# Walter0807/MotionBERT

Hardware: AMD Instinct MI355X
Metric: clips/sec [B,243,17,3] DSTformer fwd+bwd (higher is better)
Workload: dtype bf16; 1 GPU; MotionBERT full DSTformer (dim_feat 512, depth 5, 8 heads, mlp_ratio 2) train step: fwd + bwd + AdamW, 64 clips/GPU x T=243 x J=17, random-init weights, pose loss (mpjpe + 0.5 n_mpjpe + 20 velocity, fused kernel), one-launch flat AdamW; global_batch=64, frames=243, parallelism=dp1

## Files before the change

motionbert_amd/csrc/elementwise.hip:

```cpp
#include "mbx_common.h"

static thread_local char g_err[512] = "";
int mbx_set_error(const char* fmt, ...) {
    va_list ap;
    va_start(ap, fmt);
    vsnprintf(g_err, sizeof(g_err), fmt, ap);
    va_end(ap);
    return 1;
}
extern "C" const char* mbx_last_error(void) { return g_err; }

#include <atomic>
static std::atomic<uintptr_t> g_lds_key[512];
static std::atomic<size_t> g_lds_size[512];
int mbx_set_dyn_lds(const void* kernel, size_t bytes, const char* who) {
    if (bytes > 160 * 1024) return mbx_set_error("%s: needs %zu bytes of LDS (> 160 KiB)", who, bytes);
    int dev = 0;
    if (hipGetDevice(&dev) != hipSuccess) dev = 0;
    const uintptr_t key = (reinterpret_cast<uintptr_t>(kernel) << 6) ^ (uintptr_t)(dev + 1);
    int slot = (int)((key * 0x9E3779B97F4A7C15ull) >> 55);
    for (int probe = 0; probe < 512; ++probe, slot = (slot + 1) & 511) {
        uintptr_t k = g_lds_key[slot].load(std::memory_order_acquire);
        if (k == 0 && g_lds_key[slot].compare_exchange_strong(k, key, std::memory_order_acq_rel)) k = key;
        if (k != key) continue;
// ... 280 lines not shown
        const int rpp = 256 / c4n;
        const int blocks = clamp_grid((M + 4 * rpp - 1) / (4 * rpp), 256 * 8);
        int chunk = (M + blocks - 1) / blocks;
        chunk = ((chunk + 4 * rpp - 1) / (4 * rpp)) * (4 * rpp);
        const int grid = (M + chunk - 1) / chunk;
        hipLaunchKernelGGL(embed_fwd_rows_kernel, dim3(grid), dim3(256), 0, (hipStream_t)stream, x, w, b, pos, temp, h, M, T, J, Din, C, chunk);
    } else {
        const int grid = clamp_grid(((size_t)M * (C / 4) + 255) / 256, 256 * 16);
        hipLaunchKernelGGL(embed_fwd_kernel, dim3(grid), dim3(256), 0, (hipStream_t)stream, x, w, b, pos, temp, h, M, T, J, Din, C);
    }
    MBX_LAUNCH_CHECK("embed_fwd");
    return 0;
}

#define EMB_MAXDIN 4
__device__ __forceinline__ float4 embed_dh4(const float* __restrict__ dh, const bf16_t* __restrict__ dh_a, const bf16_t* __restrict__ dh_b, size_t o) {
    if (dh_a == nullptr) return *reinterpret_cast<const float4*>(dh + o);
    float u[4], v[4];
    load4<bf16_t>(dh_a + o, u);
    load4<bf16_t>(dh_b + o, v);
    return make_float4(u[0] + v[0], u[1] + v[1], u[2] + v[2], u[3] + v[3]);
}
__global__ __launch_bounds__(256) void embed_bwd_kernel(const float* __restrict__ dh, const float* __restrict__ x,
                                                        float* __restrict__ dtemp, float* __restrict__ part, int B, int T,
                                                        int J, int Din, int C, const bf16_t* __restrict__ dh_a = nullptr,
                                                        const bf16_t* __restrict__ dh_b = nullptr) {
    __shared__ float4 red[256][1 + EMB_MAXDIN];
    const int t = blockIdx.x;
    const int stride = J * C + C * Din + C;
    float* prow = part + (size_t)t * stride;
    const int nq = C / 4, ns = max(256 / nq, 1);
    for (int q0 = 0; q0 < nq; q0 += 256) {
        const int q = q0 + (int)threadIdx.x % min(nq, 256), sl = (int)threadIdx.x / min(nq, 256);
        const bool act = q < nq && sl < ns;
        const int c = q * 4;
        float4 at = make_float4(0.f, 0.f, 0.f, 0.f), aw[EMB_MAXDIN];
#pragma unroll
        for (int k = 0; k < EMB_MAXDIN; ++k) aw[k] = make_float4(0.f, 0.f, 0.f, 0.f);
        for (int j = 0; j < J; ++j) {
            float4 ap = make_float4(0.f, 0.f, 0.f, 0.f);
            if (act) {
                for (int b0 = sl; b0 < B; b0 += 8 * ns) {
                    float4 g[8];
#pragma unroll
                    for (int u = 0; u < 8; ++u) {
                        const int b = min(b0 + u * ns, B - 1);
                        g[u] = embed_dh4(dh, dh_a, dh_b, (((size_t)b * T + t) * J + j) * C + c);
                    }
#pragma unroll
                    for (int u = 0; u < 8; ++u) {
                        const int b = b0 + u * ns;
                        const float on = b < B ? 1.f : 0.f;
                        const size_t m = ((size_t)min(b, B - 1) * T + t) * J + j;
                        ap.x = fmaf(on, g[u].x, ap.x); ap.y = fmaf(on, g[u].y, ap.y); ap.z = fmaf(on, g[u].z, ap.z); ap.w = fmaf(on, g[u].w, ap.w);
#pragma unroll
                        for (int k = 0; k < EMB_MAXDIN; ++k)
                            if (k < Din) {
                                const float xv = on * x[m * Din + k];
                                aw[k].x = fmaf(g[u].x, xv, aw[k].x); aw[k].y = fmaf(g[u].y, xv, aw[k].y);
                                aw[k].z = fmaf(g[u].z, xv, aw[k].z); aw[k].w = fmaf(g[u].w, xv, aw[k].w);
                            }
                    }
                }
            }
            red[threadIdx.x][0] = ap;
            __syncthreads();
            if (act && sl == 0) {
                for (int s2 = 1; s2 < ns; ++s2) {
                    const float4 o = red[threadIdx.x + s2 * nq][0];
                    ap.x += o.x; ap.y += o.y; ap.z += o.z; ap.w += o.w;
                }
                *reinterpret_cast<float4*>(prow + (size_t)j * C + c) = ap;
                at.x += ap.x; at.y += ap.y; at.z += ap.z; at.w += ap.w;
            }
            __syncthreads();
        }
#pragma unroll
        for (int k = 0; k < EMB_MAXDIN; ++k) red[threadIdx.x][1 + k] = aw[k];
        __syncthreads();
        if (act && sl == 0) {
            *reinterpret_cast<float4*>(dtemp + (size_t)t * C + c) = at;
            *reinterpret_cast<float4*>(prow + (size_t)J * C + (size_t)C * Din + c) = at;
#pragma unroll
            for (int k = 0; k < EMB_MAXDIN; ++k)
                if (k < Din) {
                    float4 w4 = aw[k];
                    for (int s2 = 1; s2 < ns; ++s2) {
                        const float4 o = red[threadIdx.x + s2 * nq][1 + k];
                        w4.x += o.x; w4.y += o.y; w4.z += o.z; w4.w += o.w;
                    }
// ... 20 lines not shown
        for (int k = 0; k < EMB_MAXDIN; ++k) {
            const float s = wave_sum(a[k]);
            if (lane == 0 && k < Din) dx[(size_t)m * Din + k] = s;
        }
    }
}
extern "C" size_t mbx_embed_bwd_ws(int T, int J, int Din, int C) { return (size_t)T * ((size_t)J * C + (size_t)C * Din + C) * sizeof(float); }
static int launch_embed_bwd(const float* dh, const bf16_t* dh_a, const bf16_t* dh_b, const float* x, const float* w, float* dw, float* db,
                            float* dpos, float* dtemp, float* dx, int B, int T, int J, int Din, int C, void* ws, void* stream) {
    MBX_CHECK_ARG((dh || (dh_a && dh_b)) && x && w && dw && db && dpos && dtemp && ws, "embed_bwd: null pointer");
    MBX_CHECK_ARG(Din <= EMB_MAXDIN, "embed_bwd: dim_in %d > %d unsupported", Din, EMB_MAXDIN);
    MBX_CHECK_ARG(B > 0 && T > 0 && J > 0 && C > 0 && C % 4 == 0, "embed_bwd: bad shape (C %% 4 != 0?)");
    hipStream_t s = (hipStream_t)stream;
    float* part = (float*)ws;
    const int stride = J * C + C * Din + C;
    hipLaunchKernelGGL(embed_bwd_kernel, dim3(T), dim3(256), 0, s, dh, x, dtemp, part, B, T, J, Din, C, dh_a, dh_b);
    MBX_LAUNCH_CHECK("embed_bwd");
    if (mbx_launch_colsum(part, T, stride, 0, J * C, dpos, s)) return 1;
    if (mbx_launch_colsum(part, T, stride, J * C, C * Din, dw, s)) return 1;
    if (mbx_launch_colsum(part, T, stride, J * C + C * Din, C, db, s)) return 1;
    if (dx) {
        const int M = B * T * J;
        hipLaunchKernelGGL(embed_bwd_dx_kernel, dim3(clamp_grid((M + 3) / 4, 2048)), dim3(256), 0, s, dh, w, dx, M, Din, C, dh_a, dh_b);
        MBX_LAUNCH_CHECK("embed_bwd_dx");
    }
    return 0;
}
extern "C" int mbx_embed_bwd(const float* dh, const float* x, const float* w, float* dw, float* db, float* dpos,
                             float* dtemp, float* dx, int B, int T, int J, int Din, int C, void* ws, void* stream) {
    MBX_CHECK_ARG(dh, "embed_bwd: null pointer");
    return launch_embed_bwd(dh, nullptr, nullptr, x, w, dw, db, dpos, dtemp, dx, B, T, J, Din, C, ws, stream);
// ... 728 lines not shown
extern "C" int mbx_average_bwd(const float* dh, float* d_st, float* d_ts, void* d_st_t, void* d_ts_t, size_t n,
                               int dtype, void* stream) {
    MBX_CHECK_ARG(dh && d_st && d_ts && d_st_t && d_ts_t && n % 4 == 0, "average_bwd: bad arguments");
    const int grid = clamp_grid((n / 4 + 255) / 256, 4096);
    if (dtype == MBX_BF16)
        hipLaunchKernelGGL(average_bwd_kernel<bf16_t>, dim3(grid), dim3(256), 0, (hipStream_t)stream, dh, d_st, d_ts, (bf16_t*)d_st_t, (bf16_t*)d_ts_t, n / 4);
    else if (dtype == MBX_F32)
        hipLaunchKernelGGL(average_bwd_kernel<float>, dim3(grid), dim3(256), 0, (hipStream_t)stream, dh, d_st, d_ts, (float*)d_st_t, (float*)d_ts_t, n / 4);
    else
        return mbx_set_error("average_bwd: unknown dtype %d", dtype);
    MBX_LAUNCH_CHECK("average_bwd");
    return 0;
}

#define HEAD_MAXD 8
template <int VPL>
__global__ __launch_bounds__(256) void head_fwd_kernel(const float* __restrict__ rep, const float* __restrict__ w,
                                                       const float* __restrict__ b, float* __restrict__ out, int M, int R,
                                                       int Dout) {
    const int lane = threadIdx.x & 63;
    for (int row = blockIdx.x * 4 + (threadIdx.x >> 6); row < M; row += gridDim.x * 4) {
        float v[VPL][4];
        ROW_LOOP(k) {
            const int c = ROW_C(k);
            if (c < R) load4<float>(rep + (size_t)row * R + c, v[k]);
        }
        float mine = 0.f;
        for (int i = 0; i < Dout; ++i) {
            float a = 0.f;
            ROW_LOOP(k) {
                const int c = ROW_C(k);
                if (c < R) {
                    float ww[4];
                    load4<float>(w + (size_t)i * R + c, ww);
#pragma unroll
                    for (int e = 0; e < 4; ++e) a = fmaf(v[k][e], ww[e], a);
                }
            }
            a = wave_sum(a) + b[i];
            if (lane == i) mine = a;
        }
        if (lane < Dout) out[(size_t)row * Dout + lane] = mine;
    }
}
extern "C" int mbx_head_fwd(const float* rep, const float* w, const float* b, float* out, int M, int R, int Dout,
                            void* stream) {
    MBX_CHECK_ARG(rep && w && b && out, "head_fwd: null pointer");
    MBX_CHECK_ARG(M > 0 && R % 4 == 0 && Dout >= 1 && Dout <= HEAD_MAXD, "head_fwd: need R %% 4 == 0 and 1 <= dim_out <= %d", HEAD_MAXD);
    const int grid = clamp_grid((M + 3) / 4, 256 * 8);
    hipStream_t s = (hipStream_t)stream;
    DISPATCH_VPL(vpl_for(R), hipLaunchKernelGGL((head_fwd_kernel<VPL>), dim3(grid), dim3(256), 0, s, rep, w, b, out, M, R, Dout));
    MBX_LAUNCH_CHECK("head_fwd");
    return 0;
}

#define HEAD_BWD_BLOCKS 1024
template <typename T, int VPL>
// ... 3 lines not shown
    extern __shared__ __attribute__((aligned(16))) float lds[];
    const int lane = threadIdx.x & 63, wave = threadIdx.x >> 6;
    const int n = Dout * R + 8;
    float* mine = lds + (size_t)wave * n;
    constexpr int DG = 4;
    for (int i0 = 0; i0 < Dout; i0 += DG) {
        float gw[DG][VPL][4], gbv[DG];
#pragma unroll
        for (int j = 0; j < DG; ++j) {
            gbv[j] = 0.f;
            ROW_LOOP(k) {
#pragma unroll
                for (int e = 0; e < 4; ++e) gw[j][k][e] = 0.f;
            }
        }
        for (int row = blockIdx.x * 4 + wave; row < M; row += gridDim.x * 4) {
            float dvg[DG];
#pragma unroll
            for (int j = 0; j < DG; ++j) dvg[j] = i0 + j < Dout ? dout[(size_t)row * Dout + i0 + j] : 0.f;
#pragma unroll
            for (int j = 0; j < DG; ++j) gbv[j] += dvg[j];
            float dv[HEAD_MAXD];
            if (i0 == 0) {
#pragma unroll
                for (int q = 0; q < HEAD_MAXD; ++q) dv[q] = q < DG ? dvg[q < DG ? q : 0] : (q < Dout ? dout[(size_t)row * Dout + q] : 0.f);
            }
            ROW_LOOP(k) {
                const int c = ROW_C(k);
                if (c < R) {
                    float r[4];
                    load4<float>(rep + (size_t)row * R + c, r);
#pragma unroll
                    for (int j = 0; j < DG; ++j)
#pragma unroll
                        for (int e = 0; e < 4; ++e) gw[j][k][e] = fmaf(dvg[j], r[e], gw[j][k][e]);
                    if (i0 == 0) {
                        float o[4] = {0.f, 0.f, 0.f, 0.f};
#pragma unroll
                        for (int q = 0; q < HEAD_MAXD; ++q) {
                            if (q < Dout) {
                                float ww[4];
                                load4<float>(w + (size_t)q * R + c, ww);
#pragma unroll
                                for (int e = 0; e < 4; ++e) o[e] = fmaf(dv[q], ww[e], o[e]);
                            }
                        }
#pragma unroll
                        for (int e = 0; e < 4; ++e) o[e] *= (1.0f - r[e] * r[e]);
                        store4<T>(dpre + (size_t)row * R + c, o);
                    }
                }
            }
        }
#pragma unroll
        for (int j = 0; j < DG; ++j) {
            if (i0 + j < Dout) {
                ROW_LOOP(k) {
                    const int c = ROW_C(k);
                    if (c < R) store4<float>(mine + (size_t)(i0 + j) * R + c, gw[j][k]);
                }
                if (lane == 0) mine[Dout * R + i0 + j] = gbv[j];
            }
        }
    }
// ... 54 lines not shown
```

motionbert_amd/csrc/gemm_rows_n.hip:

```cpp
#include "mbx_common.h"
#include "lds_stream.h"
#include "mbx_diag.h"

#ifdef MBX_RN_TRACE
__device__ long long* g_rn_trace;
static constexpr int RN_TRACE_SLOTS = 12;
#define RN_TS(slot_) MBX_STAMP(tsr[slot_])
#else
#define RN_TS(slot_) do { } while (0)
#endif
static constexpr int RN_BM = 128;
static constexpr int RN_STAGE = 32 * 1024;
static constexpr int RN_RING = 4 * RN_STAGE;
template <int NT> struct RnGeo {
    static constexpr int N = 32 * NT, KPS = 32 / NT, TRIP = 16 / KPS, NQ = NT / 4;
    static constexpr int LA = NT == 16 ? 4 : 3, TS0 = NT == 16 ? 25 : 1;
};
__host__ __device__ constexpr int rn_cnt(int kps, int trip, int la, int ts0, bool last, int u) {
    int t_lo = 0, t_hi = 0;
    for (int j = 0; j < kps; ++j) { t_lo += ts0 + 4 * j < 27; t_hi += ts0 + 4 * j > 23; }
    const bool t2 = !last || u - 2 + la < trip, t1 = !last || u - 1 + la < trip, t0 = !last || u + la < trip;
    if (u == 0) return 8 + 2 + 6 + (t0 ? t_lo : 0);
    if (u == 1) return 2 + (8 + (t1 ? kps : 0)) + 6 + (t0 ? t_lo : 0);
    return (2 + (t2 ? t_hi : 0)) + (8 + (t1 ? kps : 0)) + (6 + (t0 ? t_lo : 0));
// ... 358 lines not shown
#pragma unroll
    for (int j = 0; j < NQ; ++j) {
#pragma unroll
        for (int r4 = 0; r4 < 8; ++r4) {
            const int rl = 4 * r4 + xr_e;
            const uint4 v = *reinterpret_cast<const uint4*>(rw + j * 32768 + r4 * 4096 + lane_e * 16);
            *reinterpret_cast<uint4*>(xhat_o + (size_t)min(mw + rl, M - 1) * RN_N + j * 128 + ((xp_e ^ (rl & 15)) << 3)) = v;
        }
    }
    if (g_e == 0 && mw + i_e < M) {
        mean_o[mw + i_e] = mu;
        rstd_o[mw + i_e] = rs;
    }
}

extern "C" size_t mbx_rows_n_pack_bytes(int N, int K) { return (size_t)N * K * sizeof(bf16_t); }

extern "C" int mbx_rows_n_pack_many(const int64_t* desc, int n_desc, int N, int max_k, void* stream) {
    MBX_CHECK_ARG(desc && n_desc > 0, "rows_n_pack_many: bad arguments");
    MBX_CHECK_ARG((N == 512 || N == 256) && max_k >= 256 && max_k % 256 == 0, "rows_n_pack_many: N=%d (256 or 512), max_k=%d (%% 256)", N, max_k);
    hipLaunchKernelGGL(rows_n_pack_many_kernel, dim3(((max_k / 16) * (N / 32) + 3) / 4, n_desc), dim3(256), 0, (hipStream_t)stream, desc, N / 32);
    MBX_LAUNCH_CHECK("rows_n_pack_many");
    return 0;
}

#define RN_CHECK_SHAPE(who_)                                                                                         \
    MBX_CHECK_ARG(M > 0 && ((N == 512 && K >= 512) || (N == 256 && K >= 256)) && K % 256 == 0,                      \
                  who_ ": bad shape M=%d N=%d (512 with K >= 512, or 256 with K >= 256) K=%d (%% 256)", M, N, K)

extern "C" int mbx_rows_lnbwd_t(const void* dy, const void* packed, const void* xhat, const float* rstd, const void* dres_t, void* dx_t,
// ... 9 lines not shown
#ifdef MBX_RN_TRACE
    mbx_diag_arm(HIP_SYMBOL(g_rn_trace), (size_t)grid * RN_TRACE_SLOTS * sizeof(long long), (hipStream_t)stream);
#endif
    if (N == 512)
        hipLaunchKernelGGL(rows_n_lnbwd_kernel<16>, dim3(grid), dim3(256), RN_RING + 4 * 8192, (hipStream_t)stream, (const bf16_t*)dy,
                           (const char*)packed, (const bf16_t*)xhat, rstd, (const bf16_t*)dres_t, (bf16_t*)dx_t, M, K);
    else
        hipLaunchKernelGGL(rows_n_lnbwd_kernel<8>, dim3(grid), dim3(256), RN_RING + 4 * 8192, (hipStream_t)stream, (const bf16_t*)dy,
                           (const char*)packed, (const bf16_t*)xhat, rstd, (const bf16_t*)dres_t, (bf16_t*)dx_t, M, K);
    MBX_LAUNCH_CHECK("rows_lnbwd_t");
    return 0;
}

extern "C" int mbx_rows_resid_ln(const void* a, const void* packed, const float* bias, const float* resid, float* y, void* xhat,
                                 float* mean, float* rstd, float eps, int M, int N, int K, void* stream) {
    MBX_CHECK_ARG(a && packed && bias && resid && y && xhat && mean && rstd, "rows_resid_ln: null pointer");
    RN_CHECK_SHAPE("rows_resid_ln");
    MBX_CHECK_ARG((size_t)M * N * 4 < ((size_t)1 << 32), "rows_resid_ln: M=%d rows of %d bytes exceed the 32-bit row offsets of the kernel", M, N * 4);
    MBX_CHECK_ARG((size_t)M * K * 2 < ((size_t)1 << 32), "rows_resid_ln: a of M=%d x K=%d exceeds the 32-bit lane offsets of the kernel", M, K);
    MBX_CHECK_ARG((const void*)y != (const void*)resid && xhat != a, "rows_resid_ln: y aliases resid (or xhat aliases a): rows past M re-read row M - 1 after it was stored");
    const void* kern = N == 512 ? reinterpret_cast<const void*>(rows_n_resid_ln_kernel<16>) : reinterpret_cast<const void*>(rows_n_resid_ln_kernel<8>);
    if (mbx_set_dyn_lds(kern, RN_RING + 4 * 8192, "rows_resid_ln")) return 1;
    if (N == 512)
        hipLaunchKernelGGL(rows_n_resid_ln_kernel<16>, dim3((M + RN_BM - 1) / RN_BM), dim3(256), RN_RING + 4 * 8192, (hipStream_t)stream, (const bf16_t*)a,
                           (const char*)packed, bias, resid, y, (bf16_t*)xhat, mean, rstd, eps, M, K);
    else
        hipLaunchKernelGGL(rows_n_resid_ln_kernel<8>, dim3((M + RN_BM - 1) / RN_BM), dim3(256), RN_RING + 4 * 8192, (hipStream_t)stream, (const bf16_t*)a,
                           (const char*)packed, bias, resid, y, (bf16_t*)xhat, mean, rstd, eps, M, K);
    MBX_LAUNCH_CHECK("rows_resid_ln");
    return 0;
}
```

motionbert_amd/engine.py:

```python
from __future__ import annotations

from collections import namedtuple
from dataclasses import dataclass
from typing import Any, ClassVar, Dict, List, Optional

import os

import torch

EPI_STORE = 0
EPI_GELU = 1
EPI_RESID = 2
EPI_TANH = 3
EPI_DGELU = 4

MODE_SPATIAL = 0
MODE_TEMPORAL = 1


@dataclass(frozen=True)
class ModelCfg:
    dim_in: int
    dim_out: int
    C: int
# ... 12 lines not shown
    dpr: tuple = ()

    @property
    def hd(self) -> int:
        return self.C // self.H


@dataclass(frozen=True)
class Switches:
    x3_planes: bool
    dual_stream: bool
    fold_ln: bool
    grad_stream: bool
    rows_lnbwd: bool
    rows_resid_ln: bool
    block_grad_t: bool
    gelu_d: bool
    rawln: bool
    proj_mlp: bool

    _ENV: ClassVar[tuple] = (('x3_planes', 'MBX_X3_PLANES', '1'), ('dual_stream', 'MBX_DUAL_STREAM', '1'),
            ('fold_ln', 'MBX_FOLD_LN', '1'), ('grad_stream', 'MBX_GRAD_STREAM', '1'),
            ('rows_lnbwd', 'MBX_ROWS_LNBWD', '1'), ('rows_resid_ln', 'MBX_ROWS_RESID_LN', '1'), ('block_grad_t', 'MBX_BLOCK_GRAD_T', '1'),
            ('gelu_d', 'MBX_GELU_D', '1'), ('rawln', 'MBX_RAWLN', '1'), ('proj_mlp', 'MBX_PROJ_MLP', '1'))

    @classmethod
    def from_env(cls, env=None) -> 'Switches':
        env = os.environ if env is None else env
        return cls(**{field: env.get(var, default) == '1' for field, var, default in cls._ENV})


SWITCHES = Switches.from_env()


def reload_switches(env=None) -> Switches:
    global SWITCHES
    SWITCHES = Switches.from_env(env)
    return SWITCHES
# ... 59 lines not shown
        self.drop_seed = drop_seed
        self.recompute = False
        self.x3 = x3
        self.x3_planes = sw.x3_planes and hasattr(ops, 'layernorm_fwd_planes_ok')
        self.Wn: Dict[str, torch.Tensor] = {}
        self.Wt: Dict[str, torch.Tensor] = {}
        self.dual = sw.dual_stream and getattr(ops, 'multi_stream', False)
        self.fold = sw.fold_ln and not x3 and drop_seed is None and self._can('can_fold')
        self.gstream_allowed = sw.grad_stream and bool(getattr(ops, 'grad_stream_t', False))
        self.gstream = False
        self.Bf: Dict[str, torch.Tensor] = {}
        self.Rs: Dict[str, torch.Tensor] = {}
        self.rows_lnbwd = sw.rows_lnbwd and self._can('can_rows_lnbwd')
        self.Pn: Dict[str, torch.Tensor] = {}
        self.rows_resid_ln = sw.rows_resid_ln and self._can('can_rows_resid_ln')
        self.Pf: Dict[str, torch.Tensor] = {}
        self.block_grad_t = sw.block_grad_t and self.rows_lnbwd and hasattr(ops, 'fuse_bwd_pair') and hasattr(ops, 'embed_bwd_pair')
        self.gelu_d = sw.gelu_d and self.rows_lnbwd and self._can('can_gelu_d')
        self.rawln = False
        self.rawln_allowed = sw.rawln
        self.Pk: Dict[str, torch.Tensor] = {}
        self.Pk_proj: Dict[str, str] = {}
        self.proj_mlp = sw.proj_mlp and hasattr(ops, 'proj_mlp_fused_fwd')

    def _streams(self):
        if not (self.dual and self.dev.type == 'cuda'):
            return None, None
        idx = self.dev.index if self.dev.index is not None else torch.cuda.current_device()
        side = Engine._side_streams.get(idx)
        if side is None:
# ... 36 lines not shown
    def _norm_in(self, x, pre, norm, ln):
        xn, mean, rstd = ln if ln is not None else self._layernorm(x, None if self.fold else f'{pre}.{norm}')
        return self._mm(xn), mean, rstd

    def _mm(self, t):
        return self.ops.split(t) if self.x3 and not isinstance(t, tuple) else t

    def _op(self, *shape):
        if self.x3 and self.x3_planes:
            return (torch.empty(shape, dtype=torch.bfloat16, device=self.dev), torch.empty(shape, dtype=torch.bfloat16, device=self.dev))
        return self._t(*shape)

    def _weight_cache_key(self, need_grad: bool):
        if need_grad or not hasattr(self.ops, 'weight_cache') or self.dev.type != 'cuda' or torch.cuda.is_current_stream_capturing():
            return None
        return (tuple((p.data_ptr(), p._version) for p in self.P.values()), self.T, self.fold, self.rawln, self.proj_mlp, self.x3, self.rows_resid_ln)

    def prepare_weights(self, need_grad: bool):
        cfg, ops, P = self.cfg, self.ops, self.P
        if need_grad and hasattr(ops, 'weight_cache') and self.dev.type == 'cuda':
            ops.weight_cache.pop(self.dev.index, None)
        key = self._weight_cache_key(need_grad)
        if key is not None:
            hit = ops.weight_cache.get(self.dev.index)
            if hit is not None and hit[0] == key and len(hit[1]) == len(P) and all(r() is p for r, p in zip(hit[1], P.values())):
                self.Wn, self.Wt, self.Bf, self.Rs, self.Pk, self.Pk_proj, self.Pf = hit[2]
                return
        self._prepare_weights(need_grad)
        if key is not None:
            import weakref
            ops.weight_cache[self.dev.index] = (key, [weakref.ref(p) for p in P.values()], (self.Wn, self.Wt, self.Bf, self.Rs, self.Pk, self.Pk_proj, self.Pf))

    def _prepare_weights(self, need_grad: bool):
        cfg, ops, P = self.cfg, self.ops, self.P
        if self.fold:
            pairs = folded_pairs(cfg)
            folded = {l for l, _ in pairs}
            self.Wn, self.Wt = ops.prep_weights(P, [n for n in linear_names(cfg) if n not in folded], self.T, need_grad)
            fn, ft, self.Bf, self.Rs = ops.fold_norm_weights(P, pairs, need_grad, self.T)
            self.Wn.update(fn)
            self.Wt.update(ft)
            if self.rows_resid_ln and not self.rawln:
                lins = [f'{pre}.{mod}.{LINEARS[typ][1]}' for pre, _, sub, typ, _, mod, _ in sublayers(cfg) if sub < 3]
                self.Pf = dict(zip(lins, ops.rows_n_pack_many([self.Wn[lin] for lin in lins])))
            if need_grad and self.rows_lnbwd and self.gstream_allowed:
                first = {f'{pre}.{mod}.qkv' for pre, _, sub, _, _, mod, _ in sublayers(cfg) if sub == 0 and not (self.block_grad_t and cfg.att_fuse)}
                lins = [lin for lin, _ in pairs if lin not in first]
                self.Pn = dict(zip(lins, ops.rows_n_pack_many([ft[lin] for lin in lins])))
            if self.rawln:
                before = None
                for blk, _, sub, typ, _, m, _ in sublayers(cfg):
                    pre = f'{blk}.{m}'
                    if typ == 'mlp' and self.proj_mlp and before is not None and before[0] == 'attn':
                        self.Pk_proj[pre] = f'{blk}.{before[1]}.proj'
                        self.Pk[pre] = ops.proj_mlp_pack_weights(self.Wn[self.Pk_proj[pre]], self.Wn[pre + '.fc1'], self.Wn[pre + '.fc2'])
                    elif typ == 'mlp':
                        self.Pk[pre] = ops.mlp_pack_weights(self.Wn[pre + '.fc1'], self.Wn[pre + '.fc2'])
                    before = (typ, m) if sub < 3 else None
# ... 96 lines not shown
            nxt = order[sub + 1][1] if sub + 1 < len(order) else None
            if typ == 'attn':
                defer = self.rawln and self.proj_mlp and sub + 1 < len(order) and order[sub + 1][0] == 'mlp'
                x, sv, ln, pend = self._attn_fwd(x, pre, norm, mod, mode, need_grad, sub, ln, nxt, defer_proj=defer)
            else:
                x, sv, ln = self._mlp_fwd(x, pre, norm, mod, need_grad, sub, ln, nxt, pending_proj=pend)
                pend = None
            svs.append(sv)
        assert pend is None, 'an attention deferred its proj to an MLP that never came'
        return x, svs

    def _resid_gemm(self, a, lin, x, dm, pre, nxt):
        cfg, ops, P = self.cfg, self.ops, self.P
        y = self._f(self.M, cfg.C)
        drop = dm is not None and dm.branch
        if self.fold and nxt is not None and lin in self.Pf and self.M < (1 << 21) and not drop:
            xn, mean, rstd = self._op(self.M, cfg.C), self._f(self.M), self._f(self.M)
            ops.rows_resid_ln(a, self.Pf[lin], P[lin + '.bias'], x, y, xn, mean, rstd, cfg.eps)
            return y, (xn, mean, rstd)
        ops.gemm_nt(a, self.Wn[lin], P[lin + '.bias'], EPI_RESID, resid=x, out_f=y)
        if drop and not self.rawln:
            ops.residual_drop(y, x, cfg.J, dm.p, dm.seed_branch, dm.p_path, dm.seed_path)
        return y, None

    def _attn_fwd(self, x, pre, norm, attn, mode, need_grad, sub=0, ln=None, nxt=None, defer_proj=False):
        cfg, ops, P = self.cfg, self.ops, self.P
        M, C = self.M, cfg.C
        qkv = self._t(M, 3 * C)
        lin = f'{pre}.{attn}.qkv'
        if self.rawln:
            xn = mean = rstd = None
# ... 268 lines not shown
```

motionbert_amd/hip_ops.py:

```python
from __future__ import annotations

import ctypes as C
import os
import threading
from itertools import accumulate
from typing import Dict, List, Optional

import torch

_HERE = os.path.dirname(os.path.abspath(__file__))
LIB_PATH = os.environ.get('MBX_LIB', os.path.join(_HERE, 'libmbx.so'))

MBX_F32, MBX_BF16, MBX_BF16_LO = 0, 1, 2
_DT = {torch.float32: MBX_F32, torch.bfloat16: MBX_BF16}

_vp, _i, _f, _sz, _i64p = C.c_void_p, C.c_int, C.c_float, C.c_size_t, C.c_void_p

SIGNATURES = {
    'mbx_last_error': (C.c_char_p, []),
    'mbx_version': (_i, []),
    'mbx_prep_weights': (_i, [_i64p, _i, _i, _i, _i, _vp]),
    'mbx_embed_fwd': (_i, [_vp] * 6 + [_i] * 5 + [_vp]),
    'mbx_embed_bwd_ws': (_sz, [_i] * 4),
    'mbx_embed_bwd': (_i, [_vp] * 8 + [_i] * 5 + [_vp, _vp]),
# ... 349 lines not shown
        key = (base == 0, N, tuple((w.data_ptr() - base, w.shape[1]) for w in ws), dev.index)
        ent = self._desc_entry('rnpack', key, build)
        flat = torch.empty(ent['total'], dtype=torch.uint8, device=dev)
        desc = ent['desc'].clone()
        desc[:, 0] += base
        desc[:, 1] += flat.data_ptr()
        self._ck(self.lib.mbx_rows_n_pack_many(desc.data_ptr(), len(ws), N, ent['max_k'], self._stream()))
        return [flat[o:o + N * w.shape[1] * 2] for w, o in zip(ws, ent['offs'])]

    def rows_lnbwd_t(self, dy_t, packed, xhat, rstd, dres_t, dx_t):
        M, K = dy_t.shape
        self._ck(self.lib.mbx_rows_lnbwd_t(_p(dy_t), _p(packed), _p(xhat), _p(rstd), _p(dres_t), _p(dx_t), M, dx_t.shape[1], K, self._stream()))

    can_rows_resid_ln = can_rows_lnbwd

    def rows_resid_ln(self, a_t, packed, bias, resid, y, xhat, mean, rstd, eps):
        M, K = a_t.shape
        self._ck(self.lib.mbx_rows_resid_ln(_p(a_t), _p(packed), _p(bias), _p(resid), _p(y), _p(xhat), _p(mean), _p(rstd), float(eps), M, y.shape[1], K,
                                            self._stream()))

    def mfma_probe(self, seconds: float = 0.25, wgs_per_cu: int = 1, device=None):
        dev = torch.device('cuda', torch.cuda.current_device()) if device is None else device
        cus = torch.cuda.get_device_properties(dev).multi_processor_count
        n_wg = cus * wgs_per_cu
        ws = torch.zeros(int(self.lib.mbx_mfma_probe_ws(n_wg)), dtype=torch.uint8, device=dev)
        flops = C.c_double(0.0)

        def run(iters):
            e0, e1 = torch.cuda.Event(enable_timing=True), torch.cuda.Event(enable_timing=True)
            e0.record()
# ... 678 lines not shown
```

Before: 575.3 clips/s.

## Prefetch embed backward loads, batch head rows, add plain residual GEMM

The embedding backward kernel now issues its dh loads several iterations ahead in a register ring and caches x rows in shared memory, so load latency overlaps with accumulation. The head forward and backward kernels process two rows per wave to reuse each weight load. A new rows_n_resid kernel writes residual plus bias GEMM output without layer-norm stats for the last sublayer, but it sits behind an env flag that is off by default. The main risks are higher register pressure from the prefetch buffers and more LDS use per block.

```diff
diff --git a/motionbert_amd/csrc/elementwise.hip b/motionbert_amd/csrc/elementwise.hip
--- a/motionbert_amd/csrc/elementwise.hip
+++ b/motionbert_amd/csrc/elementwise.hip
@@ -318,66 +318,109 @@
 }
 
 #define EMB_MAXDIN 4
-__device__ __forceinline__ float4 embed_dh4(const float* __restrict__ dh, const bf16_t* __restrict__ dh_a, const bf16_t* __restrict__ dh_b, size_t o) {
-    if (dh_a == nullptr) return *reinterpret_cast<const float4*>(dh + o);
-    float u[4], v[4];
-    load4<bf16_t>(dh_a + o, u);
-    load4<bf16_t>(dh_b + o, v);
-    return make_float4(u[0] + v[0], u[1] + v[1], u[2] + v[2], u[3] + v[3]);
-}
+#define EMB_PF 4
+#define EMB_XL_MAXP 2048
+__device__ __forceinline__ uint4 embed_dh_raw(const float* __restrict__ dh, const bf16_t* __restrict__ dh_a, const bf16_t* __restrict__ dh_b, size_t o) {
+    if (dh_a == nullptr) return *reinterpret_cast<const uint4*>(dh + o);
+    const uint2 a = *reinterpret_cast<const uint2*>(dh_a + o), b = *reinterpret_cast<const uint2*>(dh_b + o);
+    return make_uint4(a.x, a.y, b.x, b.y);
+}
+__device__ __forceinline__ float4 embed_dh_val(const uint4 r, bool pair) {
+    if (!pair) return make_float4(__uint_as_float(r.x), __uint_as_float(r.y), __uint_as_float(r.z), __uint_as_float(r.w));
+    return make_float4(__uint_as_float(r.x << 16) + __uint_as_float(r.z << 16), __uint_as_float(r.x & 0xffff0000u) + __uint_as_float(r.z & 0xffff0000u),
+                       __uint_as_float(r.y << 16) + __uint_as_float(r.w << 16), __uint_as_float(r.y & 0xffff0000u) + __uint_as_float(r.w & 0xffff0000u));
+}
+template <bool XL>
 __global__ __launch_bounds__(256) void embed_bwd_kernel(const float* __restrict__ dh, const float* __restrict__ x,
                                                         float* __restrict__ dtemp, float* __restrict__ part, int B, int T,
                                                         int J, int Din, int C, const bf16_t* __restrict__ dh_a = nullptr,
                                                         const bf16_t* __restrict__ dh_b = nullptr) {
     __shared__ float4 red[256][1 + EMB_MAXDIN];
+    __shared__ float4 xs[XL ? EMB_XL_MAXP : 1];
     const int t = blockIdx.x;
     const int stride = J * C + C * Din + C;
     float* prow = part + (size_t)t * stride;
+    const bool pair = dh_a != nullptr;
+    if constexpr (XL) {
+        for (int p = threadIdx.x; p < B * J; p += 256) {
+            const float* xp = x + (((size_t)(p / J) * T + t) * J + p % J) * Din;
+            xs[p] = make_float4(xp[0], Din > 1 ? xp[1] : 0.f, Din > 2 ? xp[2] : 0.f, Din > 3 ? xp[3] : 0.f);
+        }
+        __syncthreads();
+    }
     const int nq = C / 4, ns = max(256 / nq, 1);
+    const int ntr = (B + 8 * ns - 1) / (8 * ns), N = J * ntr;
     for (int q0 = 0; q0 < nq; q0 += 256) {
         const int q = q0 + (int)threadIdx.x % min(nq, 256), sl = (int)threadIdx.x / min(nq, 256);
         const bool act = q < nq && sl < ns;
         const int c = q * 4;
-        float4 at = make_float4(0.f, 0.f, 0.f, 0.f), aw[EMB_MAXDIN];
+        float4 at = make_float4(0.f, 0.f, 0.f, 0.f), ap = make_float4(0.f, 0.f, 0.f, 0.f), aw[EMB_MAXDIN];
 #pragma unroll
         for (int k = 0; k < EMB_MAXDIN; ++k) aw[k] = make_float4(0.f, 0.f, 0.f, 0.f);
-        for (int j = 0; j < J; ++j) {
-            float4 ap = make_float4(0.f, 0.f, 0.f, 0.f);
-            if (act) {
-                for (int b0 = sl; b0 < B; b0 += 8 * ns) {
-                    float4 g[8];
-#pragma unroll
-                    for (int u = 0; u < 8; ++u) {
-                        const int b = min(b0 + u * ns, B - 1);
-                        g[u] = embed_dh4(dh, dh_a, dh_b, (((size_t)b * T + t) * J + j) * C + c);
+        uint4 raw[EMB_PF][8];
+        auto request = [&](int n, uint4 (&r)[8]) __attribute__((always_inline)) {
+            const int j = n / ntr, b0 = sl + (n % ntr) * 8 * ns;
+#pragma unroll
+            for (int u = 0; u < 8; ++u) {
+                const int b = min(b0 + u * ns, B - 1);
+                r[u] = embed_dh_raw(dh, dh_a, dh_b, (((size_t)b * T + t) * J + j) * C + c);
+            }
+        };
+        if (act) {
+#pragma unroll
+            for (int s = 0; s < EMB_PF; ++s)
+                if (s < N) request(s, raw[s]);
+        }
+        for (int n0 = 0; n0 < N; n0 += EMB_PF) {
+#pragma unroll
+            for (int s = 0; s < EMB_PF; ++s) {
+                const int n = n0 + s;
+                if (n >= N) break;
+                const int j = n / ntr, tr = n % ntr, b0 = sl + tr * 8 * ns;
+                if (act) {
+                    if (b0 < B) {
+#pragma unroll
+                        for (int u = 0; u < 8; ++u) {
+                            const int b = b0 + u * ns;
+                            const float on = b < B ? 1.f : 0.f;
+                            const size_t m = ((size_t)min(b, B - 1) * T + t) * J + j;
+                            const float4 g = embed_dh_val(raw[s][u], pair);
+                            ap.x = fmaf(on, g.x, ap.x); ap.y = fmaf(on, g.y, ap.y); ap.z = fmaf(on, g.z, ap.z); ap.w = fmaf(on, g.w, ap.w);
+                            float xk[EMB_MAXDIN] = {0.f, 0.f, 0.f, 0.f};
+                            if constexpr (XL) {
+                                const float4 v = xs[min(b, B - 1) * J + j];
+                                xk[0] = v.x; xk[1] = v.y; xk[2] = v.z; xk[3] = v.w;
+                            } else {
+#pragma unroll
+                                for (int k = 0; k < EMB_MAXDIN; ++k)
+                                    if (k < Din) xk[k] = x[m * Din + k];
+                            }
+#pragma unroll
+                            for (int k = 0; k < EMB_MAXDIN; ++k)
+                                if (k < Din) {
+                                    const float xv = on * xk[k];
+                                    aw[k].x = fmaf(g.x, xv, aw[k].x); aw[k].y = fmaf(g.y, xv, aw[k].y);
+                                    aw[k].z = fmaf(g.z, xv, aw[k].z); aw[k].w = fmaf(g.w, xv, aw[k].w);
+                                }
+                        }
                     }
-#pragma unroll
-                    for (int u = 0; u < 8; ++u) {
-                        const int b = b0 + u * ns;
-                        const float on = b < B ? 1.f : 0.f;
-                        const size_t m = ((size_t)min(b, B - 1) * T + t) * J + j;
-                        ap.x = fmaf(on, g[u].x, ap.x); ap.y = fmaf(on, g[u].y, ap.y); ap.z = fmaf(on, g[u].z, ap.z); ap.w = fmaf(on, g[u].w, ap.w);
-#pragma unroll
-                        for (int k = 0; k < EMB_MAXDIN; ++k)
-                            if (k < Din) {
-                                const float xv = on * x[m * Din + k];
-                                aw[k].x = fmaf(g[u].x, xv, aw[k].x); aw[k].y = fmaf(g[u].y, xv, aw[k].y);
-                                aw[k].z = fmaf(g[u].z, xv, aw[k].z); aw[k].w = fmaf(g[u].w, xv, aw[k].w);
-                            }
+                    if (n + EMB_PF < N) request(n + EMB_PF, raw[s]);
+                }
+                if (tr == ntr - 1) {
+                    red[threadIdx.x][0] = ap;
+                    __syncthreads();
+                    if (act && sl == 0) {
+                        for (int s2 = 1; s2 < ns; ++s2) {
+                            const float4 o = red[threadIdx.x + s2 * nq][0];
+                            ap.x += o.x; ap.y += o.y; ap.z += o.z; ap.w += o.w;
+                        }
+                        *reinterpret_cast<float4*>(prow + (size_t)j * C + c) = ap;
+                        at.x += ap.x; at.y += ap.y; at.z += ap.z; at.w += ap.w;
                     }
+                    __syncthreads();
+                    ap = make_float4(0.f, 0.f, 0.f, 0.f);
                 }
             }
-            red[threadIdx.x][0] = ap;
-            __syncthreads();
-            if (act && sl == 0) {
-                for (int s2 = 1; s2 < ns; ++s2) {
-                    const float4 o = red[threadIdx.x + s2 * nq][0];
-                    ap.x += o.x; ap.y += o.y; ap.z += o.z; ap.w += o.w;
-                }
-                *reinterpret_cast<float4*>(prow + (size_t)j * C + c) = ap;
-                at.x += ap.x; at.y += ap.y; at.z += ap.z; at.w += ap.w;
-            }
-            __syncthreads();
         }
 #pragma unroll
         for (int k = 0; k < EMB_MAXDIN; ++k) red[threadIdx.x][1 + k] = aw[k];
@@ -428,7 +471,10 @@
     hipStream_t s = (hipStream_t)stream;
     float* part = (float*)ws;
     const int stride = J * C + C * Din + C;
-    hipLaunchKernelGGL(embed_bwd_kernel, dim3(T), dim3(256), 0, s, dh, x, dtemp, part, B, T, J, Din, C, dh_a, dh_b);
+    if ((size_t)B * J <= EMB_XL_MAXP && Din >= 1)
+        hipLaunchKernelGGL(embed_bwd_kernel<true>, dim3(T), dim3(256), 0, s, dh, x, dtemp, part, B, T, J, Din, C, dh_a, dh_b);
+    else
+        hipLaunchKernelGGL(embed_bwd_kernel<false>, dim3(T), dim3(256), 0, s, dh, x, dtemp, part, B, T, J, Din, C, dh_a, dh_b);
     MBX_LAUNCH_CHECK("embed_bwd");
     if (mbx_launch_colsum(part, T, stride, 0, J * C, dpos, s)) return 1;
     if (mbx_launch_colsum(part, T, stride, J * C, C * Din, dw, s)) return 1;
@@ -1187,33 +1233,53 @@
 }
 
 #define HEAD_MAXD 8
+template <int VPL> struct HeadRows { static constexpr int RPW = VPL <= 4 ? 2 : 1; };
 template <int VPL>
 __global__ __launch_bounds__(256) void head_fwd_kernel(const float* __restrict__ rep, const float* __restrict__ w,
                                                        const float* __restrict__ b, float* __restrict__ out, int M, int R,
                                                        int Dout) {
-    const int lane = threadIdx.x & 63;
-    for (int row = blockIdx.x * 4 + (threadIdx.x >> 6); row < M; row += gridDim.x * 4) {
-        float v[VPL][4];
-        ROW_LOOP(k) {
-            const int c = ROW_C(k);
-            if (c < R) load4<float>(rep + (size_t)row * R + c, v[k]);
-        }
-        float mine = 0.f;
+    constexpr int RPW = HeadRows<VPL>::RPW;
+    const int lane = threadIdx.x & 63, step = gridDim.x * 4;
+    for (int row0 = blockIdx.x * 4 + (threadIdx.x >> 6); row0 < M; row0 += step * RPW) {
+        float v[RPW][VPL][4];
+#pragma unroll
+        for (int u = 0; u < RPW; ++u) {
+            const int row = min(row0 + u * step, M - 1);
+            ROW_LOOP(k) {
+                const int c = ROW_C(k);
+                if (c < R) load4<float>(rep + (size_t)row * R + c, v[u][k]);
+            }
+        }
+        float mine[RPW];
+#pragma unroll
+        for (int u = 0; u < RPW; ++u) mine[u] = 0.f;
         for (int i = 0; i < Dout; ++i) {
-            float a = 0.f;
+            float a[RPW];
+#pragma unroll
+            for (int u = 0; u < RPW; ++u) a[u] = 0.f;
             ROW_LOOP(k) {
                 const int c = ROW_C(k);
                 if (c < R) {
                     float ww[4];
                     load4<float>(w + (size_t)i * R + c, ww);
 #pragma unroll
-                    for (int e = 0; e < 4; ++e) a = fmaf(v[k][e], ww[e], a);
+                    for (int u = 0; u < RPW; ++u)
+#pragma unroll
+                        for (int e = 0; e < 4; ++e) a[u] = fmaf(v[u][k][e], ww[e], a[u]);
                 }
             }
-            a = wave_sum(a) + b[i];
-            if (lane == i) mine = a;
-        }
-        if (lane < Dout) out[(size_t)row * Dout + lane] = mine;
+            const float bi = b[i];
+#pragma unroll
+            for (int u = 0; u < RPW; ++u) {
+                a[u] = wave_sum(a[u]) + bi;
+                if (lane == i) mine[u] = a[u];
+            }
+        }
+#pragma unroll
+        for (int u = 0; u < RPW; ++u) {
+            const int row = row0 + u * step;
+            if (row < M && lane < Dout) out[(size_t)row * Dout + lane] = mine[u];
+        }
     }
 }
 extern "C" int mbx_head_fwd(const float* rep, const float* w, const float* b, float* out, int M, int R, int Dout,
@@ -1247,40 +1313,66 @@
                 for (int e = 0; e < 4; ++e) gw[j][k][e] = 0.f;
             }
         }
-        for (int row = blockIdx.x * 4 + wave; row < M; row += gridDim.x * 4) {
-            float dvg[DG];
-#pragma unroll
-            for (int j = 0; j < DG; ++j) dvg[j] = i0 + j < Dout ? dout[(size_t)row * Dout + i0 + j] : 0.f;
-#pragma unroll
-            for (int j = 0; j < DG; ++j) gbv[j] += dvg[j];
-            float dv[HEAD_MAXD];
+        constexpr int RPW = HeadRows<VPL>::RPW;
+        const int step = gridDim.x * 4;
+        for (int row0 = blockIdx.x * 4 + wave; row0 < M; row0 += step * RPW) {
+            float dvg[RPW][DG], r[RPW][VPL][4];
+#pragma unroll
+            for (int u = 0; u < RPW; ++u) {
+                const int row = min(row0 + u * step, M - 1);
+#pragma unroll
+                for (int j = 0; j < DG; ++j) dvg[u][j] = i0 + j < Dout ? dout[(size_t)row * Dout + i0 + j] : 0.f;
+                ROW_LOOP(k) {
+                    const int c = ROW_C(k);
+                    if (c < R) load4<float>(rep + (size_t)row * R + c, r[u][k]);
+                }
+            }
+#pragma unroll
+            for (int u = 0; u < RPW; ++u) {
+                if (row0 + u * step < M) {
+#pragma unroll
+                    for (int j = 0; j < DG; ++j) gbv[j] += dvg[u][j];
+                    ROW_LOOP(k) {
+                        if (ROW_C(k) < R) {
+#pragma unroll
+                            for (int j = 0; j < DG; ++j)
+#pragma unroll
+                                for (int e = 0; e < 4; ++e) gw[j][k][e] = fmaf(dvg[u][j], r[u][k][e], gw[j][k][e]);
+                        }
+                    }
+                }
+            }
             if (i0 == 0) {
-#pragma unroll
-                for (int q = 0; q < HEAD_MAXD; ++q) dv[q] = q < DG ? dvg[q < DG ? q : 0] : (q < Dout ? dout[(size_t)row * Dout + q] : 0.f);
-            }
-            ROW_LOOP(k) {
-                const int c = ROW_C(k);
-                if (c < R) {
-                    float r[4];
-                    load4<float>(rep + (size_t)row * R + c, r);
-#pragma unroll
-                    for (int j = 0; j < DG; ++j)
-#pragma unroll
-                        for (int e = 0; e < 4; ++e) gw[j][k][e] = fmaf(dvg[j], r[e], gw[j][k][e]);
-                    if (i0 == 0) {
-                        float o[4] = {0.f, 0.f, 0.f, 0.f};
+                ROW_LOOP(k) {
+                    const int c = ROW_C(k);
+                    if (c < R) {
+                        float o[RPW][4];
+#pragma unroll
+                        for (int u = 0; u < RPW; ++u)
+#pragma unroll
+                            for (int e = 0; e < 4; ++e) o[u][e] = 0.f;
 #pragma unroll
                         for (int q = 0; q < HEAD_MAXD; ++q) {
                             if (q < Dout) {
                                 float ww[4];
                                 load4<float>(w + (size_t)q * R + c, ww);
 #pragma unroll
-                                for (int e = 0; e < 4; ++e) o[e] = fmaf(dv[q], ww[e], o[e]);
+                                for (int u = 0; u < RPW; ++u) {
+                                    const float d = q < DG ? dvg[u][q < DG ? q : 0] : dout[(size_t)min(row0 + u * step, M - 1) * Dout + q];
+#pragma unroll
+                                    for (int e = 0; e < 4; ++e) o[u][e] = fmaf(d, ww[e], o[u][e]);
+                                }
                             }
                         }
 #pragma unroll
-                        for (int e = 0; e < 4; ++e) o[e] *= (1.0f - r[e] * r[e]);
-                        store4<T>(dpre + (size_t)row * R + c, o);
+                        for (int u = 0; u < RPW; ++u) {
+                            const int row = row0 + u * step;
+                            if (row < M) {
+#pragma unroll
+                                for (int e = 0; e < 4; ++e) o[u][e] *= (1.0f - r[u][k][e] * r[u][k][e]);
+                                store4<T>(dpre + (size_t)row * R + c, o[u]);
+                            }
+                        }
                     }
                 }
             }
diff --git a/motionbert_amd/csrc/gemm_rows_n.hip b/motionbert_amd/csrc/gemm_rows_n.hip
--- a/motionbert_amd/csrc/gemm_rows_n.hip
+++ b/motionbert_amd/csrc/gemm_rows_n.hip
@@ -396,6 +396,89 @@
     }
 }
 
+template <int NT>
+__global__ __launch_bounds__(256, 1) void rows_n_resid_kernel(const bf16_t* __restrict__ a, const char* __restrict__ wpk,
+                                                             const float* __restrict__ bias, const float* __restrict__ resid,
+                                                             float* __restrict__ y, int M, int K) {
+    constexpr int RN_N = RnGeo<NT>::N, NQ = RnGeo<NT>::NQ;
+    extern __shared__ __attribute__((aligned(16))) char ring[];
+    const int tid = threadIdx.x, lane = tid & 63, wave = __builtin_amdgcn_readfirstlane(tid >> 6);
+    const int i = lane & 31, g = lane >> 5;
+    const int mw = blockIdx.x * RN_BM + 32 * wave;
+    const unsigned dlu = __builtin_amdgcn_readfirstlane((unsigned)(uintptr_t)(const lds_void_t*)ring + wave * 1024);
+    const unsigned aoff = ((unsigned)min(mw + i, M - 1) * (unsigned)K + 8u * g) * 2u;
+    u32x4_t bq0, bq1;
+    {
+        const float* const bp = bias + (lane & (RN_N / 8 - 1)) * 8;
+        asm volatile("global_load_dwordx4 %0, %1, off" : "=v"(bq0) : "v"(bp) : "memory");
+        asm volatile("global_load_dwordx4 %0, %1, off offset:16" : "=v"(bq1) : "v"(bp) : "memory");
+    }
+    unsigned doff[16];
+#pragma unroll
+    for (int d = 0; d < 16; ++d) doff[d] = (unsigned)min(mw + 2 * d + g, M - 1) * (RN_N * 4) + ((i ^ (2 * d + g)) << 4);
+    f32x16_t acc[NT];
+    rn_product<NT, 16 * NQ>(acc, reinterpret_cast<const char*>(a), aoff, wpk, ring, dlu, K, [] {},
+                            [&](auto n, auto sp) __attribute__((always_inline)) {
+                                rn_glds<decltype(sp)::value>(reinterpret_cast<const char*>(resid) + (n >> 4) * 512, doff[n & 15], dlu);
+                            });
+    asm volatile("s_waitcnt lgkmcnt(0)" : "+v"(bq0), "+v"(bq1) : : "memory");
+    __builtin_amdgcn_s_barrier();
+    if (MBX_RN_DBG & 1) return;
+#pragma unroll
+    for (int t = 0; t < NT; ++t) MFMA_PAD_A(acc[t]);
+
+    int tid_e = threadIdx.x;
+    asm volatile("" : "+v"(tid_e));
+    const int lane_e = tid_e & 63, i_e = lane_e & 31, g_e = lane_e >> 5;
+    char* const rw = ring + wave * 1024;
+    char* const bx = ring + RN_RING + wave * 8192;
+    const unsigned rwl = __builtin_amdgcn_readfirstlane((unsigned)(uintptr_t)(const lds_void_t*)ring + wave * 1024);
+    unsigned doff_e[16];
+#pragma unroll
+    for (int d = 0; d < 16; ++d) {
+        const int rl = 2 * d + g_e;
+        doff_e[d] = (unsigned)min(mw + rl, M - 1) * (RN_N * 4) + ((i_e ^ rl) << 4);
+    }
+    RN_RDMA(1, 1, 10);
+    asm volatile("s_waitcnt vmcnt(16)" ::: "memory");
+    *reinterpret_cast<u32x4_t*>(bx + lane_e * 32) = bq0;
+    *reinterpret_cast<u32x4_t*>(bx + lane_e * 32 + 16) = bq1;
+    char* const rb_i = rw + (i_e >> 4) * 32768 + ((i_e >> 1) & 7) * 4096 + (i_e & 1) * 512;
+    const int sx = i_e << 4;
+#pragma unroll
+    for (int j = 0; j < NQ; ++j) {
+        if (j >= 1) { if (j + 1 < NQ) rn_vmwait<32>(); else rn_vmwait<16>(); }
+        char* const rbj = rb_i + (j & 1) * 65536;
+        float4 rq[2][4], bq[2][4];
+#pragma unroll
+        for (int qq = 0; qq < 4; ++qq) { rq[0][qq] = RN_RRD(0, qq); bq[0][qq] = RN_BRD(0, qq); }
+#pragma unroll
+        for (int ntl = 0; ntl < 4; ++ntl) {
+            if (ntl + 1 < 4) {
+#pragma unroll
+                for (int qq = 0; qq < 4; ++qq) { rq[(ntl + 1) & 1][qq] = RN_RRD(ntl + 1, qq); bq[(ntl + 1) & 1][qq] = RN_BRD(ntl + 1, qq); }
+            }
+            f32x16_t t = acc[4 * j + ntl];
+#pragma unroll
+            for (int qq = 0; qq < 4; ++qq) {
+                float4* const p = reinterpret_cast<float4*>(rbj + (((8 * ntl + 2 * qq + g_e) << 4) ^ sx));
+                const float4 r = rq[ntl & 1][qq], b = bq[ntl & 1][qq];
+                t[4 * qq] += r.x + b.x; t[4 * qq + 1] += r.y + b.y; t[4 * qq + 2] += r.z + b.z; t[4 * qq + 3] += r.w + b.w;
+                *p = make_float4(t[4 * qq], t[4 * qq + 1], t[4 * qq + 2], t[4 * qq + 3]);
+            }
+            __builtin_amdgcn_sched_barrier(0);
+        }
+        asm volatile("s_waitcnt lgkmcnt(0)" ::: "memory");
+#pragma unroll
+        for (int d = 0; d < 16; ++d) {
+            const float4 v = *reinterpret_cast<const float4*>(RN_RCH(j & 1, d) + lane_e * 16);
+            *reinterpret_cast<float4*>(reinterpret_cast<char*>(y) + doff_e[d] + j * 512) = v;
+        }
+        asm volatile("s_waitcnt lgkmcnt(0)" ::: "memory");
+        if (j + 2 < NQ) { if (j == 0) { RN_RDMA(2, 0, 0); } else if (j == 1) { RN_RDMA(3, 1, 0); } }
+    }
+}
+
 extern "C" size_t mbx_rows_n_pack_bytes(int N, int K) { return (size_t)N * K * sizeof(bf16_t); }
 
 extern "C" int mbx_rows_n_pack_many(const int64_t* desc, int n_desc, int N, int max_k, void* stream) {
@@ -435,11 +518,25 @@
 
 extern "C" int mbx_rows_resid_ln(const void* a, const void* packed, const float* bias, const float* resid, float* y, void* xhat,
                                  float* mean, float* rstd, float eps, int M, int N, int K, void* stream) {
-    MBX_CHECK_ARG(a && packed && bias && resid && y && xhat && mean && rstd, "rows_resid_ln: null pointer");
+    MBX_CHECK_ARG(a && packed && bias && resid && y, "rows_resid_ln: null pointer");
+    const bool plain = !xhat && !mean && !rstd;
+    MBX_CHECK_ARG(plain || (xhat && mean && rstd), "rows_resid_ln: xhat, mean and rstd are all NULL (y alone) or all given");
     RN_CHECK_SHAPE("rows_resid_ln");
     MBX_CHECK_ARG((size_t)M * N * 4 < ((size_t)1 << 32), "rows_resid_ln: M=%d rows of %d bytes exceed the 32-bit row offsets of the kernel", M, N * 4);
     MBX_CHECK_ARG((size_t)M * K * 2 < ((size_t)1 << 32), "rows_resid_ln: a of M=%d x K=%d exceeds the 32-bit lane offsets of the kernel", M, K);
     MBX_CHECK_ARG((const void*)y != (const void*)resid && xhat != a, "rows_resid_ln: y aliases resid (or xhat aliases a): rows past M re-read row M - 1 after it was stored");
+    if (plain) {
+        const void* kp = N == 512 ? reinterpret_cast<const void*>(rows_n_resid_kernel<16>) : reinterpret_cast<const void*>(rows_n_resid_kernel<8>);
+        if (mbx_set_dyn_lds(kp, RN_RING + 4 * 8192, "rows_resid_ln")) return 1;
+        if (N == 512)
+            hipLaunchKernelGGL(rows_n_resid_kernel<16>, dim3((M + RN_BM - 1) / RN_BM), dim3(256), RN_RING + 4 * 8192, (hipStream_t)stream, (const bf16_t*)a,
+                               (const char*)packed, bias, resid, y, M, K);
+        else
+            hipLaunchKernelGGL(rows_n_resid_kernel<8>, dim3((M + RN_BM - 1) / RN_BM), dim3(256), RN_RING + 4 * 8192, (hipStream_t)stream, (const bf16_t*)a,
+                               (const char*)packed, bias, resid, y, M, K);
+        MBX_LAUNCH_CHECK("rows_resid_ln");
+        return 0;
+    }
     const void* kern = N == 512 ? reinterpret_cast<const void*>(rows_n_resid_ln_kernel<16>) : reinterpret_cast<const void*>(rows_n_resid_ln_kernel<8>);
     if (mbx_set_dyn_lds(kern, RN_RING + 4 * 8192, "rows_resid_ln")) return 1;
     if (N == 512)
diff --git a/motionbert_amd/engine.py b/motionbert_amd/engine.py
--- a/motionbert_amd/engine.py
+++ b/motionbert_amd/engine.py
@@ -50,6 +50,7 @@
     grad_stream: bool
     rows_lnbwd: bool
     rows_resid_ln: bool
+    rows_resid_plain: bool
     block_grad_t: bool
     gelu_d: bool
     rawln: bool
@@ -57,7 +58,8 @@
 
     _ENV: ClassVar[tuple] = (('x3_planes', 'MBX_X3_PLANES', '1'), ('dual_stream', 'MBX_DUAL_STREAM', '1'),
             ('fold_ln', 'MBX_FOLD_LN', '1'), ('grad_stream', 'MBX_GRAD_STREAM', '1'),
-            ('rows_lnbwd', 'MBX_ROWS_LNBWD', '1'), ('rows_resid_ln', 'MBX_ROWS_RESID_LN', '1'), ('block_grad_t', 'MBX_BLOCK_GRAD_T', '1'),
+            ('rows_lnbwd', 'MBX_ROWS_LNBWD', '1'), ('rows_resid_ln', 'MBX_ROWS_RESID_LN', '1'),
+            ('rows_resid_plain', 'MBX_ROWS_RESID_PLAIN', '0'), ('block_grad_t', 'MBX_BLOCK_GRAD_T', '1'),
             ('gelu_d', 'MBX_GELU_D', '1'), ('rawln', 'MBX_RAWLN', '1'), ('proj_mlp', 'MBX_PROJ_MLP', '1'))
 
     @classmethod
@@ -147,6 +149,7 @@
         self.rows_lnbwd = sw.rows_lnbwd and self._can('can_rows_lnbwd')
         self.Pn: Dict[str, torch.Tensor] = {}
         self.rows_resid_ln = sw.rows_resid_ln and self._can('can_rows_resid_ln')
+        self.rows_resid_plain = sw.rows_resid_plain and self.rows_resid_ln and self._can('can_rows_resid_plain')
         self.Pf: Dict[str, torch.Tensor] = {}
         self.block_grad_t = sw.block_grad_t and self.rows_lnbwd and hasattr(ops, 'fuse_bwd_pair') and hasattr(ops, 'embed_bwd_pair')
         self.gelu_d = sw.gelu_d and self.rows_lnbwd and self._can('can_gelu_d')
@@ -213,7 +216,7 @@
     def _weight_cache_key(self, need_grad: bool):
         if need_grad or not hasattr(self.ops, 'weight_cache') or self.dev.type != 'cuda' or torch.cuda.is_current_stream_capturing():
             return None
-        return (tuple((p.data_ptr(), p._version) for p in self.P.values()), self.T, self.fold, self.rawln, self.proj_mlp, self.x3, self.rows_resid_ln)
+        return (tuple((p.data_ptr(), p._version) for p in self.P.values()), self.T, self.fold, self.rawln, self.proj_mlp, self.x3, self.rows_resid_ln, self.rows_resid_plain)
 
     def prepare_weights(self, need_grad: bool):
         cfg, ops, P = self.cfg, self.ops, self.P
@@ -240,7 +243,8 @@
             self.Wn.update(fn)
             self.Wt.update(ft)
             if self.rows_resid_ln and not self.rawln:
-                lins = [f'{pre}.{mod}.{LINEARS[typ][1]}' for pre, _, sub, typ, _, mod, _ in sublayers(cfg) if sub < 3]
+                nsub = 4 if self.rows_resid_plain else 3
+                lins = [f'{pre}.{mod}.{LINEARS[typ][1]}' for pre, _, sub, typ, _, mod, _ in sublayers(cfg) if sub < nsub]
                 self.Pf = dict(zip(lins, ops.rows_n_pack_many([self.Wn[lin] for lin in lins])))
             if need_grad and self.rows_lnbwd and self.gstream_allowed:
                 first = {f'{pre}.{mod}.qkv' for pre, _, sub, _, _, mod, _ in sublayers(cfg) if sub == 0 and not (self.block_grad_t and cfg.att_fuse)}
@@ -367,7 +371,10 @@
         cfg, ops, P = self.cfg, self.ops, self.P
         y = self._f(self.M, cfg.C)
         drop = dm is not None and dm.branch
-        if self.fold and nxt is not None and lin in self.Pf and self.M < (1 << 21) and not drop:
+        if self.fold and lin in self.Pf and self.M < (1 << 21) and not drop:
+            if nxt is None:
+                ops.rows_resid_ln(a, self.Pf[lin], P[lin + '.bias'], x, y, None, None, None, cfg.eps)
+                return y, None
             xn, mean, rstd = self._op(self.M, cfg.C), self._f(self.M), self._f(self.M)
             ops.rows_resid_ln(a, self.Pf[lin], P[lin + '.bias'], x, y, xn, mean, rstd, cfg.eps)
             return y, (xn, mean, rstd)
diff --git a/motionbert_amd/hip_ops.py b/motionbert_amd/hip_ops.py
--- a/motionbert_amd/hip_ops.py
+++ b/motionbert_amd/hip_ops.py
@@ -387,6 +387,8 @@
 
     can_rows_resid_ln = can_rows_lnbwd
 
+    can_rows_resid_plain = can_rows_lnbwd
+
     def rows_resid_ln(self, a_t, packed, bias, resid, y, xhat, mean, rstd, eps):
         M, K = a_t.shape
         self._ck(self.lib.mbx_rows_resid_ln(_p(a_t), _p(packed), _p(bias), _p(resid), _p(y), _p(xhat), _p(mean), _p(rstd), float(eps), M, y.shape[1], K,
```

Result: no change. 579.2 clips/s (median of 6 runs) (+0.7%).
